# roboterax/humanoid-gym

Hardware: AMD Instinct MI355X
Metric: env-steps/s (XBot-L PPO, whole job) (higher is better)
Workload: dtype bf16

## Files before the change

### humanoid-gym_amd/csrc/hgym_fused.hpp

```cpp
#pragma once
#include "hgym_finalize.hpp"
#pragma clang fp contract(fast)
#include "hgym_gemm.hpp"

namespace hgym {

constexpr int FUSED_CHUNK = 128;

struct __attribute__((packed, aligned(4))) F4 {
    float v[4];
};
typedef __attribute__((ext_vector_type(4))) short s16x4;
typedef __attribute__((ext_vector_type(2))) unsigned int u32x2;

struct FusedLayer {
    const u32x4* Wf;
    const u32x4* WTf;
    const float* bias;
    int K, N;
    int KB;
    int NB;
    int NBB;
};

// ... 607 lines not shown
        stage_load(c0);
        hook_early(extra);
        stage_write(c0, 0);
        bias_to_lds();
        if constexpr (PART) {
#pragma unroll
            for (int i = 0; i < MB; ++i)
#pragma unroll
                for (int g = 0; g < G1; ++g)
#pragma unroll
                    for (int e = 0; e < 4; ++e) acc[i][g][e] = drop[i] ? 0.0f : acc[i][g][e];
        }
        __syncthreads();
        phase_stamp(a.dbg, 1);
        for (int c = c0; c + 1 < NC; ++c) {
            stage_load(c + 1);
            mma_chunk<G1, MB, D, false, XBF>(r0, wl0, L0.KB * 64, (c - c0) * 4, Q + ((c - c0) & 1) * (BM * FUSED_CHUNK * 2), 8, lane, acc);
            stage_write(c + 1, (c + 1 - c0) & 1);
            __syncthreads();
        }
        mma_chunk<G1, MB, D, true, XBF>(r0, wl0, L0.KB * 64, (NC - 1 - c0) * 4, Q + ((NC - 1 - c0) & 1) * (BM * FUSED_CHUNK * 2), 8, lane, acc);
        phase_stamp(a.dbg, 2);
        if (AHEAD) prime1();
        epilogue_elu<G1, MB, GA>(acc, bl, nb0, P, L0.NB, train_h ? n.H[0] : nullptr, mbg0, lane, a.act);
    }
    __syncthreads();
    phase_stamp(a.dbg, 3);
    hook_mid(extra);
    if (!AHEAD) prime1();
    auto prime2 = [&]() { hidden_prime<GH, D>(r2, L2, wave, lane); };
    hidden_layer<GH, MB, NW, D, AHEAD, GA>(r1, L1, bl + L0.N, P, L0.NB, Q, train_h ? n.H[1] : nullptr, mbg0, wave, lane, prime2, a.act);
    __syncthreads();
    phase_stamp(a.dbg, 4);
    if (!AHEAD) prime2();
    WRing<1, 4> r3;
    auto prime3 = [&]() {
        if (wave < MB) wring_prime<1, 4>(r3, L3.Wf + lane, 0, L3.KB);
    };
    hidden_layer<GH, MB, NW, D, AHEAD, GA>(r2, L2, bl + L0.N + L1.N, Q, L1.NB, PH2, train_h ? n.H[2] : nullptr, mbg0, wave, lane, prime3, a.act);
    if (wave * GH >= L2.NB) hook_l2idle(extra);
    __syncthreads();
    phase_stamp(a.dbg, 5);
    if (!AHEAD) prime3();
    if (wave < MB) {
        f32x4 hacc[1][1];
        hacc[0][0] = (f32x4){0.f, 0.f, 0.f, 0.f};
        const int CB3 = L2.NB;
        if (L3.KB % 4 == 0) mma_stream<1, 1, 4>(r3, L3.Wf + lane, 0, L3.KB, PH2 + wave * CB3 * 512, CB3, lane, hacc);
        else mma_ring<1, 1, 4>(r3, L3.Wf + lane, 0, 0, L3.KB, L3.KB, PH2 + wave * CB3 * 512, CB3, lane, hacc);
        const f32x4 acc = hacc[0][0];
        const int m = m0 + wave * 16 + r;
        const int No = L3.N;
        float mu[4];
#pragma unroll
        for (int e = 0; e < 4; ++e) mu[e] = acc[e] + ((4 * q + e < No) ? bl[L0.N + L1.N + L2.N + 4 * q + e] : 0.0f);
        if (m < a.M && n.out) {
#pragma unroll
            for (int e = 0; e < 4; ++e)
                if (4 * q + e < No) n.out[(int64_t)m * n.ldo + 4 * q + e] = mu[e];
        }
        hook_head(wave, m, 0, mu);
        if (is_actor && a.sample) {
#pragma clang fp contract(off)
            const int A = a.A;
            float zz[4];
            if (a.z) {
#pragma unroll
                for (int e = 0; e < 4; ++e) zz[e] = (m < a.M && 4 * q + e < A) ? a.z[(int64_t)m * A + 4 * q + e] : 0.0f;
            } else {
                const int64_t s = HOIST ? step_pre : (a.step ? a.step[0] : 0);
                const RngKey rk = {a.k0, a.k1, (uint32_t)s, (uint32_t)(s >> 32)};
                const U4 u = rng4(rk, (uint32_t)m, SLOT_POLICY + (uint32_t)q);
                box_muller(u.x, u.y, zz[0], zz[1]);
                box_muller(u.z, u.w, zz[2], zz[3]);
            }
            float lp = 0.0f;
#pragma unroll
            for (int e = 0; e < 4; ++e) {
                const int j = 4 * q + e;
                if (j < A) {
                    const float sg = mu[e] * 0.0f + (HOIST ? std_pre[e] : a.std_[j]);
                    const float act = mu[e] + sg * zz[e];
                    const float d = act - mu[e];
                    lp += -(d * d) / (2.0f * sg * sg) - (HOIST ? lsg_pre[e] : log_sigma(sg)) - 0.9189385332046727f;
                    if (m < a.M) {
                        a.actions[(int64_t)m * A + j] = act;
                        a.sigma[(int64_t)m * A + j] = sg;
                    }
                    hook_put(wave * 16 + r, j, act);
                }
            }
            lp += __shfl_xor(lp, 16, 64);
            lp += __shfl_xor(lp, 32, 64);
            if (q == 0 && m < a.M) a.logp[m] = lp;
        }
        for (int nb = 1; WIDE && nb < L3.NB; ++nb) {
            const u32x4* wl = L3.Wf + (int64_t)nb * L3.KB * 64 + lane;
            wring_prime<1, 4>(r3, wl, 0, L3.KB);
            hacc[0][0] = (f32x4){0.f, 0.f, 0.f, 0.f};
            if (L3.KB % 4 == 0) mma_stream<1, 1, 4>(r3, wl, 0, L3.KB, PH2 + wave * CB3 * 512, CB3, lane, hacc);
            else mma_ring<1, 1, 4>(r3, wl, 0, 0, L3.KB, L3.KB, PH2 + wave * CB3 * 512, CB3, lane, hacc);
            float y[4];
#pragma unroll
            for (int e = 0; e < 4; ++e) {
                const int col = nb * 16 + 4 * q + e;
                y[e] = hacc[0][0][e] + (col < No ? bl[L0.N + L1.N + L2.N + col] : 0.0f);
            }
            if (m < a.M && n.out) {
#pragma unroll
                for (int e = 0; e < 4; ++e)
                    if (nb * 16 + 4 * q + e < No) n.out[(int64_t)m * n.ldo + nb * 16 + 4 * q + e] = y[e];
            }
            hook_head(wave, m, nb, y);
        }
    } else {
        hook_idle(extra);
    }
    phase_stamp(a.dbg, 6);
}

template <int BM, int NW, int D, bool FIN = false>
__global__ __launch_bounds__(NW * 64) void mlp_fwd_kernel(const FwdArgs a) {
    extern __shared__ __attribute__((aligned(16))) char smem[];
    if (FIN && (int)blockIdx.y >= a.nets) {
        if (blockIdx.x == 0) fin_block(a.fin, threadIdx.x, NW * 64);
        return;
    }
    const int which = a.net0 + blockIdx.y;
    const FusedNet& n = a.net[which];
    const int g1 = n.layer[0].NB / NW;
    constexpr int U = 16 / NW;
    if (n.layer[3].NB > 1) {
        if (g1 == 2 * U) fwd_body<BM, NW, D, 2 * U, true>(a, n, false, smem);
        return;
    }
    if (g1 == 2 * U) fwd_body<BM, NW, D, 2 * U>(a, n, which == 0, smem);
    else if (g1 == 3 * U) fwd_body<BM, NW, D, 3 * U>(a, n, which == 0, smem);
    else if (g1 == U) fwd_body<BM, NW, D, U>(a, n, which == 0, smem);
}

template <int BM, int NW, int D, int G1U, bool WIDE>
__global__ __launch_bounds__(NW * 64) void mlp_fwd_act_kernel(const FwdArgs a) {
    extern __shared__ __attribute__((aligned(16))) char smem[];
    constexpr int U = 16 / NW;
    fwd_body<BM, NW, D, G1U * U, WIDE, false, false, true>(a, a.net[a.net0], !WIDE && a.net0 == 0, smem);
}

template <int G, int D, int GR>
__device__ __forceinline__ void bwd_prime(WRing<GR, D>& R, const u32x4* __restrict__ WTf, int NBo, int NBBc, int wave, int lane) {
    const int nb0 = wave * G;
    if (nb0 < NBo) wring_prime<G, D>(R, WTf + (int64_t)nb0 * NBBc * 64 + lane, NBBc * 64, NBBc);
}

template <int G, int MB, int NW, int D, bool AHEAD, bool HLDS = false, bool GA = false, int GR, class Next>
__device__ __forceinline__ void bwd_step(WRing<GR, D>& R, const u32x4* __restrict__ WTf, int NBo, int NBBc, const char* in_lds, int CBin,
                                         char* out_lds, __bf16* __restrict__ dZg, const __bf16* __restrict__ Hg, int64_t mbg0, int wave,
                                         int lane, Next prime_next, const char* H_lds = nullptr, const Act* fn = nullptr) {
    const int r = lane & 15, q = lane >> 4;
    float d0p = 0.f, d1p = 0.f, d0n = 0.f, d1n = 0.f, ndq = 0.f;
    if constexpr (GA) { d0p = fn->d0p; d1p = fn->d1p; d0n = fn->d0n; d1n = fn->d1n; ndq = -fn->dq; }
    const int loff = r * 32 + q * 8;
    bool primed = false;
    for (int nb0 = wave * G; nb0 < NBo; nb0 += NW * G) {
        f32x4 acc[MB][G];
        zero_acc<G, MB>(acc);
        if (NBBc % D == 0) mma_stream<G, MB, D>(R, WTf + (int64_t)nb0 * NBBc * 64 + lane, NBBc * 64, NBBc, in_lds, CBin, lane, acc);
        else mma_ring<G, MB, D>(R, WTf + (int64_t)nb0 * NBBc * 64 + lane, NBBc * 64, 0, NBBc, NBBc, in_lds, CBin, lane, acc);
        const int nxt = nb0 + NW * G;
        if (nxt < NBo) wring_prime<G, D>(R, WTf + (int64_t)nxt * NBBc * 64 + lane, NBBc * 64, NBBc);
        else if (AHEAD) { prime_next(); primed = true; }
        u32x2 aux[MB][G];
#pragma unroll
        for (int i = 0; i < MB; ++i)
#pragma unroll
            for (int g = 0; g < G; ++g) {
                if (HLDS) aux[i][g] = *reinterpret_cast<const u32x2*>(H_lds + (i * NBo + nb0 + g) * 512 + loff);
                else aux[i][g] = ld_stream_u2<(kFusedNT & 4) != 0>(reinterpret_cast<const char*>(Hg) + ((mbg0 + i) * NBo + nb0 + g) * 512 + loff);
            }
        static_assert(MB % 2 == 0, "row blocks are stored in pairs");
#pragma unroll
        for (int i = 0; i < MB; i += 2)
#pragma unroll
            for (int g = 0; g < G; ++g) {
                u32x2 pk[2];
#pragma unroll
                for (int h = 0; h < 2; ++h) {
                    const unsigned int w0 = aux[i + h][g][0], w1 = aux[i + h][g][1];
                    const float y[4] = {bf16_bits_to_f32(w0 & 0xffffu), bf16_bits_to_f32(w0 >> 16), bf16_bits_to_f32(w1 & 0xffffu),
                                        bf16_bits_to_f32(w1 >> 16)};
                    float d[4];
                    if constexpr (GA) {
#pragma unroll
                        for (int e = 0; e < 4; ++e) {
                            const bool p = y[e] > 0.0f;
                            d[e] = acc[i + h][g][e] * fmaf(y[e], fmaf(ndq, y[e], p ? d1p : d1n), p ? d0p : d0n);
                        }
                    } else {
#pragma unroll
                        for (int e = 0; e < 4; ++e) d[e] = acc[i + h][g][e] * ((y[e] > 0.0f) ? 1.0f : (y[e] + 1.0f));
                    }
                    pk[h] = pack_bf16x4(d[0], d[1], d[2], d[3]);
                    if (out_lds) *reinterpret_cast<u32x2*>(out_lds + ((i + h) * NBo + nb0 + g) * 512 + loff) = pk[h];
                }
                char* pa = reinterpret_cast<char*>(dZg) + ((mbg0 + i) * NBo + nb0 + g) * 512 + loff;
                st_pair<(kFusedNT & 4) != 0, false>(pa, pa + (int64_t)NBo * 512, pk[0], pk[1], true, true, q);
            }
    }
    if (AHEAD && !primed) prime_next();
}

struct FbLoss {
    const float* actions;
    const float* old_mu;
    const float* old_sigma;
    const float* values;
    const float* advantages;
    const float* returns;
    const float* logp;
    float clip, value_coef, entropy_coef;
    float* partials;
    const float* aux_target;
    int64_t aux_ldt;
    int aux_off;
    float aux_coef;
};

constexpr int FB_LIN_ACTOR = 40;
HG_HD int fb_lds_lin(const FusedNet& n) { return n.layer[3].N == 1 ? 64 * 2 * 4 : (n.layer[3].N <= 12 ? 64 * FB_LIN_ACTOR * 4 : 0); }
HG_HD int fb_lds_extra(const FusedNet& n) { return 64 * 64 * n.layer[3].NBB + 4 * 32 * 4 + 64 * n.layer[2].N * 2 + 256 + fb_lds_lin(n); }

constexpr size_t FB_LDS_LIMIT = 160 * 1024;
HG_HD int fwd_lds_bytes(const FusedNet& n, int BM) { return fused_lds_p(n, BM) + fused_lds_q(n, BM) + fused_lds_bias(n); }
HG_HD int fb_lds_bytes(const FusedNet& n) { return fwd_lds_bytes(n, 64) + fb_lds_extra(n); }
inline int fb_lds_bytes(const int32_t* dims) {
    FusedNet n{};
    for (int l = 0; l < 4; ++l) {
        n.layer[l].K = dims[l];
        n.layer[l].N = dims[l + 1];
        n.layer[l].NB = (dims[l + 1] + 15) / 16;
        n.layer[l].NBB = (dims[l + 1] + 31) / 32;
    }
    return fb_lds_bytes(n);
}

template <int G1, bool AUX = false, bool XB16 = false, bool VU = false, bool GA = false>
__device__ __forceinline__ void fb_body(const FwdArgs& a, const FbLoss& L, const FusedNet& n, bool is_actor, char* smem) {
    constexpr int BM = 64, NW = 16, D = 2, MB = BM / 16;
    const int tid = threadIdx.x, lane = tid & 63, wave = tid >> 6;
    const int r = lane & 15, q = lane >> 4;
    const int m0 = blockIdx.x * BM;
    const int64_t mbg0 = m0 >> 4;
    char* P = smem;
    char* Q = smem + fused_lds_p(n, BM);
    char* R0 = smem + fused_lds_p(n, BM) + fused_lds_q(n, BM) + fused_lds_bias(n);
    const int NBB3 = n.layer[3].NBB, CB3 = 2 * NBB3;
    float* red = reinterpret_cast<float*>(R0 + BM * 64 * NBB3);
    char* H2 = R0 + BM * 64 * NBB3 + 4 * 32 * 4;
    int* rowidx = reinterpret_cast<int*>(H2 + BM * n.layer[2].N * 2);
    float* lin = reinterpret_cast<float*>(rowidx + BM);
    const int A = a.A;
    const bool pre = !AUX && n.layer[2].NB <= 8 && (is_actor ? A == 12 : true);
    const float invB = 1.0f / (float)a.M;
    float aux_se = 0.0f;
    auto head_aux = [&](int hw, int m, int nb, const float (&out)[4]) {
        const int No = n.layer[3].N;
        const bool valid = m < a.M;
        const int64_t row = rowidx[hw * 16 + r];
        const float* t = L.aux_target + row * L.aux_ldt + L.aux_off;
        const float gs = 2.0f * L.aux_coef / ((float)a.M * (float)No);
        float g[4];
#pragma unroll
        for (int e = 0; e < 4; ++e) {
            const int j = nb * 16 + 4 * q + e;
            float d = 0.0f;
            if (valid && j < No) {
                d = out[e] - t[j];
                aux_se += d * d;
            }
            g[e] = gs * d;
        }
        const u32x2 pk = pack_bf16x4(g[0], g[1], g[2], g[3]);
        const int off = (hw * CB3 + nb) * 512 + r * 32 + q * 8;
        char* gz = reinterpret_cast<char*>(n.dZ[3]) + mbg0 * CB3 * 512;
        *reinterpret_cast<u32x2*>(R0 + off) = pk;
        *reinterpret_cast<u32x2*>(gz + off) = pk;
        if (nb == 0) {
            const u32x2 zero = {0u, 0u};
            for (int cb = n.layer[3].NB; cb < CB3; ++cb) {
                const int offz = (hw * CB3 + cb) * 512 + r * 32 + q * 8;
                *reinterpret_cast<u32x2*>(R0 + offz) = zero;
                *reinterpret_cast<u32x2*>(gz + offz) = zero;
            }
        }
    };
    auto l2idle = [&](int) {
        if (!pre) return;
        const int j = tid - 8 * 64;
        if (j < 0) return;
        if (is_actor) {
            const int rw = j >> 3, k = j & 7;
            const int64_t ri = rowidx[rw];
            const float* base = k < 3 ? L.actions : (k < 6 ? L.old_mu : L.old_sigma);
            const F4 v1 = *reinterpret_cast<const F4*>(base + ri * 12 + 4 * (k < 3 ? k : (k < 6 ? k - 3 : k - 6)));
            const int rw2 = j & 63;
            const int64_t ri2 = rowidx[rw2];
            const F4 v2 = *reinterpret_cast<const F4*>(L.old_sigma + ri2 * 12 + 8);
            const float s2 = (j < 128 ? L.advantages : L.logp)[ri2];
            *reinterpret_cast<F4*>(lin + rw * FB_LIN_ACTOR + 4 * k) = v1;
            if (j < 64) *reinterpret_cast<F4*>(lin + rw2 * FB_LIN_ACTOR + 32) = v2;
            else if (j < 192) lin[rw2 * FB_LIN_ACTOR + (j < 128 ? 36 : 37)] = s2;
        } else if (j < 128) {
            const int rw = j & 63;
            const int64_t ri = rowidx[rw];
            lin[rw * 2 + (j >> 6)] = j < 64 ? L.returns[ri] : L.values[ri];
        }
    };
    auto head = [&](int hw, int m, int, const float (&out)[4]) {
        const bool valid = m < a.M;
        const int rl = hw * 16 + r;
        const int64_t row = rowidx[rl];
        float g[4] = {0.f, 0.f, 0.f, 0.f};
        float part[11];
#pragma unroll
        for (int k = 0; k < 11; ++k) part[k] = 0.0f;
        if (is_actor) {
            float act[4] = {0.f, 0.f, 0.f, 0.f}, mo[4] = {0.f, 0.f, 0.f, 0.f}, so[4] = {1.f, 1.f, 1.f, 1.f}, sg[4] = {1.f, 1.f, 1.f, 1.f};
            if (pre) {
                if (q < 3) {
                    const F4 qa = *reinterpret_cast<const F4*>(lin + rl * FB_LIN_ACTOR + 4 * q);
                    const F4 qo = *reinterpret_cast<const F4*>(lin + rl * FB_LIN_ACTOR + 12 + 4 * q);
                    const F4 qs = *reinterpret_cast<const F4*>(lin + rl * FB_LIN_ACTOR + 24 + 4 * q);
#pragma unroll
                    for (int e = 0; e < 4; ++e) { act[e] = qa.v[e]; mo[e] = qo.v[e]; so[e] = qs.v[e]; }
                }
            } else if (4 * q + 3 < A) {
                const F4 qa = *reinterpret_cast<const F4*>(L.actions + row * A + 4 * q);
                const F4 qo = *reinterpret_cast<const F4*>(L.old_mu + row * A + 4 * q);
                const F4 qs = *reinterpret_cast<const F4*>(L.old_sigma + row * A + 4 * q);
#pragma unroll
                for (int e = 0; e < 4; ++e) { act[e] = qa.v[e]; mo[e] = qo.v[e]; so[e] = qs.v[e]; }
            } else {
#pragma unroll
                for (int e = 0; e < 4; ++e)
                    if (4 * q + e < A) { act[e] = L.actions[row * A + 4 * q + e]; mo[e] = L.old_mu[row * A + 4 * q + e]; so[e] = L.old_sigma[row * A + 4 * q + e]; }
            }
            const float adv = pre ? lin[rl * FB_LIN_ACTOR + 36] : L.advantages[row], lpold = pre ? lin[rl * FB_LIN_ACTOR + 37] : L.logp[row];
            float lp = 0.0f, ent = 0.0f, kl = 0.0f, diff[4];
#pragma unroll
            for (int e = 0; e < 4; ++e) {
                diff[e] = 0.0f;
                if (4 * q + e < A) {
                    const float mm = out[e];
                    const float s = mm * 0.0f + a.std_[4 * q + e];
                    const float d = act[e] - mm;
                    diff[e] = d;
                    sg[e] = s;
                    lp += -(d * d) / (2.0f * s * s) - logf(s) - 0.9189385332046727f;
                    ent += 0.5f + 0.9189385332046727f + logf(s);
                    kl += logf(s / so[e] + 1.e-5f) + (so[e] * so[e] + (mo[e] - mm) * (mo[e] - mm)) / (2.0f * (s * s)) - 0.5f;
                }
            }
            lp += __shfl_xor(lp, 16, 64);  lp += __shfl_xor(lp, 32, 64);
            ent += __shfl_xor(ent, 16, 64); ent += __shfl_xor(ent, 32, 64);
            kl += __shfl_xor(kl, 16, 64);  kl += __shfl_xor(kl, 32, 64);
            const float ratio = expf(lp - lpold);
            const float s1 = -adv * ratio;
            const float s2 = -adv * clampf(ratio, 1.0f - L.clip, 1.0f + L.clip);
            const float in_range = (ratio >= 1.0f - L.clip && ratio <= 1.0f + L.clip) ? 1.0f : 0.0f;
            const float w1 = s1 > s2 ? 1.0f : (s1 == s2 ? 0.5f : 0.0f);
            const float d_lp = (-adv) * (w1 + (1.0f - w1) * in_range) * invB * ratio;
            if (valid) {
                if (q == 0) { part[0] = fmaxf(s1, s2); part[1] = ent; part[2] = kl; }
#pragma unroll
                for (int e = 0; e < 4; ++e)
                    if (4 * q + e < A) {
                        const float s = sg[e], d = diff[e];
                        g[e] = d_lp * d / (s * s);
                        part[3 + e] = d_lp * (d * d / (s * s * s) - 1.0f / s) - (L.entropy_coef * invB) / s;
                        part[7 + e] = g[e];
                    }
            }
        } else {
            const float ret = pre ? lin[rl * 2] : L.returns[row], vold = pre ? lin[rl * 2 + 1] : L.values[row];
            const float v = out[0];
            if constexpr (VU) {
                (void)vold;
                if (valid && q == 0) {
                    g[0] = L.value_coef * invB * (2.0f * (v - ret));
                    part[0] = (v - ret) * (v - ret);
                    part[1] = g[0];
                }
            } else {
                const float vc = vold + clampf(v - vold, -L.clip, L.clip);
                const float l1 = (v - ret) * (v - ret), l2 = (vc - ret) * (vc - ret);
                const float v_in = ((v - vold) >= -L.clip && (v - vold) <= L.clip) ? 1.0f : 0.0f;
                const float u1 = l1 > l2 ? 1.0f : (l1 == l2 ? 0.5f : 0.0f);
                if (valid && q == 0) {
                    g[0] = L.value_coef * invB * (u1 * 2.0f * (v - ret) + (1.0f - u1) * 2.0f * (vc - ret) * v_in);
                    part[0] = fmaxf(l1, l2);
                    part[1] = g[0];
                }
            }
        }
        const u32x2 pk = pack_bf16x4(g[0], g[1], g[2], g[3]);
        const u32x2 zero = {0u, 0u};
        const int off0 = (hw * 2 + 0) * 512 + r * 32 + q * 8, off1 = (hw * 2 + 1) * 512 + r * 32 + q * 8;
        *reinterpret_cast<u32x2*>(R0 + off0) = pk;
        *reinterpret_cast<u32x2*>(R0 + off1) = zero;
        char* gz = reinterpret_cast<char*>(n.dZ[3]) + mbg0 * 2 * 512;
        *reinterpret_cast<u32x2*>(gz + off0) = pk;
        *reinterpret_cast<u32x2*>(gz + off1) = zero;
#pragma unroll
        for (int k = 0; k < 11; ++k) {
            float v = part[k];
            v += __shfl_xor(v, 1, 64); v += __shfl_xor(v, 2, 64); v += __shfl_xor(v, 4, 64); v += __shfl_xor(v, 8, 64);
            part[k] = v;
        }
        if (r == 0) {
            float* w = red + hw * 32;
            if (is_actor) {
                if (q == 0) { w[0] = part[0]; w[2] = part[1]; w[3] = part[2]; }
#pragma unroll
                for (int e = 0; e < 4; ++e)
                    if (4 * q + e < 12) { w[4 + 4 * q + e] = part[3 + e]; w[16 + 4 * q + e] = part[7 + e]; }
            } else if (q == 0) {
                w[1] = part[0];
                w[28] = part[1];
            }
        }
    };
    if constexpr (AUX) {
        fwd_body<BM, NW, D, G1, true, XB16, false, GA>(a, n, false, smem, FwdNoop(), FwdNoop(), FwdNoop(), 0, FwdNoop(), head_aux, H2, rowidx);
        if (wave < MB) {
#pragma unroll
            for (int o = 32; o > 0; o >>= 1) aux_se += __shfl_xor(aux_se, o, 64);
            if (lane == 0) red[wave * 32 + 29] = aux_se;
        }
    } else {
        fwd_body<BM, NW, D, G1, false, XB16, false, GA>(a, n, is_actor, smem, FwdNoop(), FwdNoop(), FwdNoop(), 0, FwdNoop(), head, H2, rowidx, l2idle);
    }
    __syncthreads();
    if (tid < 32) {
        const bool mine = AUX ? tid == 29 : (is_actor ? (tid != 1 && tid < 28) : (tid == 1 || tid == 28));
        if (mine) L.partials[(int64_t)blockIdx.x * 32 + tid] = red[tid] + red[32 + tid] + red[64 + tid] + red[96 + tid];
    }
    const int N0 = n.layer[0].N, N1 = n.layer[1].N, N2 = n.layer[2].N;
    WRing<1, D> ra;
    WRing<1, D> rb;
    WRing<G1, D> rc;
    auto none = [&]() {};
    bwd_prime<1, D>(ra, n.layer[3].WTf, N2 / 16, NBB3, wave, lane);
    bwd_step<1, MB, NW, D, false, true, GA>(ra, n.layer[3].WTf, N2 / 16, NBB3, R0, 2 * NBB3, H2, n.dZ[2], nullptr, mbg0, wave, lane, none, H2, &a.act);
    __syncthreads();
    bwd_prime<1, D>(rb, n.layer[2].WTf, N1 / 16, n.layer[2].NBB, wave, lane);
    bwd_step<1, MB, NW, D, false, true, GA>(rb, n.layer[2].WTf, N1 / 16, n.layer[2].NBB, H2, N2 / 16, Q, n.dZ[1], nullptr, mbg0, wave, lane, none, Q, &a.act);
    __syncthreads();
    bwd_prime<G1, D>(rc, n.layer[1].WTf, N0 / 16, n.layer[1].NBB, wave, lane);
    bwd_step<G1, MB, NW, D, false, true, GA>(rc, n.layer[1].WTf, N0 / 16, n.layer[1].NBB, Q, N1 / 16, nullptr, n.dZ[0], nullptr, mbg0, wave, lane, none, P, &a.act);
    phase_stamp(a.dbg, 7);
}

template <bool XB16 = false, bool VU = false>
__global__ __launch_bounds__(1024) void mlp_fb_kernel(const FwdArgs a, const FbLoss L) {
    extern __shared__ __attribute__((aligned(16))) char smem[];
    const int which = a.net0 + blockIdx.y;
    const FusedNet& n = a.net[which];
    const int g1 = n.layer[0].NB / 16;
    if (which == 2) {
        if (g1 == 2) fb_body<2, true, XB16, VU>(a, L, n, false, smem);
        return;
    }
    if (g1 == 2) fb_body<2, false, XB16, VU>(a, L, n, which == 0, smem);
    else if (g1 == 3) fb_body<3, false, XB16, VU>(a, L, n, which == 0, smem);
    else if (g1 == 1) fb_body<1, false, XB16, VU>(a, L, n, which == 0, smem);
}

template <bool VU>
int32_t launch_mlp_fb_form(const FwdArgs& fb, const FbLoss& fl, bool shadow, int tiles, int nets, size_t lds, hipStream_t s) {
    const int32_t rc = shadow ? ensure_dynamic_lds(reinterpret_cast<const void*>(&mlp_fb_kernel<true, VU>), lds, "mlp_fb_kernel<shadow>")
                              : ensure_dynamic_lds(reinterpret_cast<const void*>(&mlp_fb_kernel<false, VU>), lds, "mlp_fb_kernel");
    if (rc) return rc;
    if (shadow) hipLaunchKernelGGL((mlp_fb_kernel<true, VU>), dim3(tiles, nets), dim3(1024), lds, s, fb, fl);
    else hipLaunchKernelGGL((mlp_fb_kernel<false, VU>), dim3(tiles, nets), dim3(1024), lds, s, fb, fl);
    return HGYM_OK;
}

template <int G1, bool AUX, bool XB16, bool VU>
__global__ __launch_bounds__(1024) void mlp_fb_act_kernel(const FwdArgs a, const FbLoss L) {
    extern __shared__ __attribute__((aligned(16))) char smem[];
    fb_body<G1, AUX, XB16, VU, true>(a, L, a.net[a.net0], !AUX && a.net0 == 0, smem);
}

template <int G1, bool AUX, bool VU>
int32_t launch_mlp_fb_act_one(const FwdArgs& fb, const FbLoss& fl, bool shadow, int tiles, size_t lds, hipStream_t s) {
    const int32_t rc = shadow ? ensure_dynamic_lds(reinterpret_cast<const void*>(&mlp_fb_act_kernel<G1, AUX, true, VU>), lds, "mlp_fb_act_kernel<shadow>")
                              : ensure_dynamic_lds(reinterpret_cast<const void*>(&mlp_fb_act_kernel<G1, AUX, false, VU>), lds, "mlp_fb_act_kernel");
    if (rc) return rc;
    if (shadow) hipLaunchKernelGGL((mlp_fb_act_kernel<G1, AUX, true, VU>), dim3(tiles), dim3(1024), lds, s, fb, fl);
    else hipLaunchKernelGGL((mlp_fb_act_kernel<G1, AUX, false, VU>), dim3(tiles), dim3(1024), lds, s, fb, fl);
    return HGYM_OK;
}
template <bool VU>
int32_t launch_mlp_fb_act_form(const FwdArgs& fb0, const FbLoss& fl, bool shadow, int tiles, int nets, hipStream_t s) {
    for (int i = 0; i < nets; ++i) {
        FwdArgs fb = fb0;
        fb.net0 = i;
        fb.nets = 1;
        if (fb.dbg) fb.dbg += (int64_t)i * tiles * 8;
        const size_t lds = (size_t)fb_lds_bytes(fb.net[i]);
        const int g1 = fb.net[i].layer[0].NB / 16;
        int32_t rc = HGYM_E_UNSUPPORTED;
        if (i == 2) rc = launch_mlp_fb_act_one<2, true, VU>(fb, fl, shadow, tiles, lds, s);
        else if (g1 == 1) rc = launch_mlp_fb_act_one<1, false, VU>(fb, fl, shadow, tiles, lds, s);
        else if (g1 == 2) rc = launch_mlp_fb_act_one<2, false, VU>(fb, fl, shadow, tiles, lds, s);
        else if (g1 == 3) rc = launch_mlp_fb_act_one<3, false, VU>(fb, fl, shadow, tiles, lds, s);
        if (rc) return rc;
    }
    return HGYM_OK;
}

constexpr int LOSS_PARTIALS = 32;
struct ScalArgs {
    int nblocks, B, A, aux_No;
    const float* partials;
    float* grads_std;
    float* grads_bmu;
    float* grads_bv;
    float* kl_slot;
    double* opt;
    double beta1, beta2;
    int do_prologue, adaptive_lr;
    float desired_kl;
    double lr_min, lr_max;
    int group;
};
__device__ __forceinline__ double adapt_lr(double lr, float kl, float desired_kl, double lr_min, double lr_max) {
    if (kl > desired_kl * 2.0f) return fmax(lr_min, lr / 1.5);
    if (kl < desired_kl * 0.5f && kl > 0.0f) return fmin(lr_max, lr * 1.5);
    return lr;
}
__device__ __forceinline__ void ppo_scalars_block(const ScalArgs& a, int tid, int nthreads) {
    __shared__ double red[16][LOSS_PARTIALS + 1];
    if (tid >= nthreads - 2 && !(a.opt[13] == a.opt[1] && a.opt[1] > 0.0)) {
        const double t = a.opt[1] + 1.0;
        const double pw = pow(tid == nthreads - 2 ? a.beta1 : a.beta2, t);
        a.opt[tid == nthreads - 2 ? 14 : 15] = pw;
        if (tid == nthreads - 2) a.opt[13] = t;
    }
    const float* __restrict__ partials = a.partials;
    const int nblocks = a.nblocks, B = a.B, A = a.A;
    const int k = tid & (LOSS_PARTIALS - 1);
    for (int part = tid / LOSS_PARTIALS; part < 16; part += nthreads / LOSS_PARTIALS) {
        double s0 = 0.0, s1 = 0.0, s2 = 0.0, s3 = 0.0;
        int b = part;
        if (a.group == 4) {
            auto ld = [&](int g) -> float {
                const float* p = partials + (int64_t)g * 4 * LOSS_PARTIALS + k;
                const float p0 = p[0], p1 = p[LOSS_PARTIALS], p2 = p[2 * LOSS_PARTIALS], p3 = p[3 * LOSS_PARTIALS];
                return ((p0 + p1) + p2) + p3;
            };
            for (; b + 48 < nblocks; b += 64) {
                const float v0 = ld(b), v1 = ld(b + 16), v2 = ld(b + 32), v3 = ld(b + 48);
                s0 += (double)v0; s1 += (double)v1; s2 += (double)v2; s3 += (double)v3;
            }
            for (; b < nblocks; b += 16) s0 += (double)ld(b);
        } else {
            for (; b + 48 < nblocks; b += 64) {
                const float v0 = partials[(int64_t)b * LOSS_PARTIALS + k], v1 = partials[(int64_t)(b + 16) * LOSS_PARTIALS + k];
                const float v2 = partials[(int64_t)(b + 32) * LOSS_PARTIALS + k], v3 = partials[(int64_t)(b + 48) * LOSS_PARTIALS + k];
                s0 += (double)v0; s1 += (double)v1; s2 += (double)v2; s3 += (double)v3;
            }
            for (; b < nblocks; b += 16) s0 += (double)partials[(int64_t)b * LOSS_PARTIALS + k];
        }
        red[part][k] = (s0 + s1) + (s2 + s3);
    }
    __syncthreads();
    if (tid < LOSS_PARTIALS) {
        double t = 0.0;
        for (int p = 0; p < 16; ++p) t += red[p][tid];
        const int q = tid;
        double* __restrict__ opt = a.opt;
        if (q == 0) opt[3] += t / B;
        if (q == 1) opt[4] += t / B;
        if (q == 2) opt[5] += t / B;
        if (q == 3) {
            const float kl = (float)(t / B);
            opt[2] += t / B;
            opt[8] = (double)kl;
            opt[7] += 1.0;
            opt[9] = 0.0;
            a.kl_slot[0] = kl;
            if (a.do_prologue && !(opt[13] == opt[1] && opt[1] > 0.0)) {
                double lr = opt[0];
                if (a.adaptive_lr) {
                    lr = adapt_lr(lr, kl, a.desired_kl, a.lr_min, a.lr_max);
                    opt[0] = lr;
                }
                const double ts = opt[1] + 1.0;
                opt[1] = ts;
                const double bc1 = 1.0 - opt[14], bc2 = 1.0 - opt[15];
                opt[11] = (double)(float)(lr / bc1);
                opt[12] = (double)(float)sqrt(bc2);
            }
        }
        if (q >= 4 && q < 16 && q - 4 < A) a.grads_std[q - 4] = (float)t;
        if (q >= 16 && q < 28 && q - 16 < A && a.grads_bmu) a.grads_bmu[q - 16] = (float)t;
        if (q == 28 && a.grads_bv) a.grads_bv[0] = (float)t;
        if (q == 29 && a.aux_No > 0) opt[10] += t / ((double)B * (double)a.aux_No);
    }
}

constexpr int DW_THREADS = 512;
constexpr int DW_Z_BYTES = 8192;
constexpr int DW_STAGE_BYTES = 24576;
constexpr int DW_LDS_STAGES = 3;
constexpr int DW_TILE_N = 128, DW_TILE_K = 256;
constexpr int DW_MAX_PRODUCTS = 12;

struct DwProduct {
    const __bf16* Z;
    const __bf16* X;
    const int64_t* gidx;
    int64_t ldg;
    int CBz, CBx;
    int N, K;
    int64_t w_off;
    int64_t b_off;
    int tiles_n, tiles_k, tile0;
};

struct DwArgs {
    DwProduct p[DW_MAX_PRODUCTS];
    int np;
    int total_tiles;
    int splits;
    int steps_total;
    int steps_per_split;
    float* slabs;
    int64_t slab_stride;
    const char* zeros;
    int B;
    int scal_bid;
    ScalArgs sc;
};

__device__ __forceinline__ u32x4 tr_frag(const char* p0, const char* p1) {
    typedef s16x4 __attribute__((address_space(3)))* lds_p;
    const s16x4 a = __builtin_amdgcn_ds_read_tr16_b64_v4i16((lds_p)(const_cast<char*>(p0)));
    const s16x4 b = __builtin_amdgcn_ds_read_tr16_b64_v4i16((lds_p)(const_cast<char*>(p1)));
    struct { s16x4 a, b; } pr = {a, b};
    return __builtin_bit_cast(u32x4, pr);
}

template <int DW_RS>
__global__ __launch_bounds__(DW_THREADS, 1) void dw_kernel_rs(const DwArgs a) {
    static_assert(DW_RS == 3, "ring indices below: three register stages over three LDS stages, unrolled by six");
    extern __shared__ __attribute__((aligned(16))) char smem[];
    const int tid = threadIdx.x, lane = tid & 63, wave = tid >> 6;
    const int wi = wave >> 1, wj = wave & 1;
    const int r = lane & 15, q = lane >> 4;
    const int bid = blockIdx.x;
    if (bid == a.scal_bid) {
        ppo_scalars_block(a.sc, tid, DW_THREADS);
        return;
    }
    const int xcd = bid & 7, slot = bid >> 3;
    const int split = xcd + 8 * (slot / a.total_tiles);
    const int tile = slot % a.total_tiles;
// ... 157 lines not shown
```

### humanoid-gym_amd/csrc/hgym_update.hip

```cpp
#include "hgym_fused.hpp"

namespace hgym {

int32_t launch_mlp_fb_unclipped(const FwdArgs& fb, const FbLoss& fl, bool shadow, int tiles, int nets, size_t lds, hipStream_t s);

int32_t launch_mlp_fb(const FwdArgs& fb, const FbLoss& fl, bool shadow, bool unclipped, int tiles, int nets, size_t lds, hipStream_t s) {
    if (unclipped) return launch_mlp_fb_unclipped(fb, fl, shadow, tiles, nets, lds, s);
    return launch_mlp_fb_form<false>(fb, fl, shadow, tiles, nets, lds, s);
}

}
```

### humanoid-gym_amd/csrc/hgym_update_act.hip

```cpp
#include "hgym_fused.hpp"

namespace hgym {

int32_t launch_mlp_fb_act_unclipped(const FwdArgs& fb, const FbLoss& fl, bool shadow, int tiles, int nets, hipStream_t s);

int32_t launch_mlp_fb_act(const FwdArgs& fb, const FbLoss& fl, bool shadow, bool unclipped, int tiles, int nets, hipStream_t s) {
    if (unclipped) return launch_mlp_fb_act_unclipped(fb, fl, shadow, tiles, nets, s);
    return launch_mlp_fb_act_form<false>(fb, fl, shadow, tiles, nets, s);
}

}
```

Measured before the change: 42.14 million.

## Fuse last-layer backward into loss head and prefetch next backward weights

For the PPO fused forward/backward kernel, the output layer's dZ computation (a single-block MMA against preloaded transposed head weights) is moved into the per-wave loss head, so it is no longer a separate backward step behind a block barrier. While the forward pass is idle, the weight ring for the next backward layer is primed, and the first-layer ring priming is chained into the second step for small G1. This is meant to shorten the serialized backward tail and remove one __syncthreads. It adds register pressure (eight held weight fragments) and an env-gated fallback path built in separate translation units for shapes that do not match.

```diff
diff --git a/humanoid-gym_amd/csrc/hgym_fused.hpp b/humanoid-gym_amd/csrc/hgym_fused.hpp
--- a/humanoid-gym_amd/csrc/hgym_fused.hpp
+++ b/humanoid-gym_amd/csrc/hgym_fused.hpp
@@ -783,13 +783,39 @@
     if (nb0 < NBo) wring_prime<G, D>(R, WTf + (int64_t)nb0 * NBBc * 64 + lane, NBBc * 64, NBBc);
 }
 
+struct ActD {
+    float d0p, d1p, d0n, d1n, ndq;
+};
+template <bool GA>
+__device__ __forceinline__ ActD act_d(const Act* fn) {
+    ActD k = {0.f, 0.f, 0.f, 0.f, 0.f};
+    if constexpr (GA) { k.d0p = fn->d0p; k.d1p = fn->d1p; k.d0n = fn->d0n; k.d1n = fn->d1n; k.ndq = -fn->dq; }
+    return k;
+}
+template <bool GA>
+__device__ __forceinline__ u32x2 dz_block(const f32x4& acc, u32x2 y2, const ActD& k) {
+    const unsigned int w0 = y2[0], w1 = y2[1];
+    const float y[4] = {bf16_bits_to_f32(w0 & 0xffffu), bf16_bits_to_f32(w0 >> 16), bf16_bits_to_f32(w1 & 0xffffu), bf16_bits_to_f32(w1 >> 16)};
+    float d[4];
+    if constexpr (GA) {
+#pragma unroll
+        for (int e = 0; e < 4; ++e) {
+            const bool p = y[e] > 0.0f;
+            d[e] = acc[e] * fmaf(y[e], fmaf(k.ndq, y[e], p ? k.d1p : k.d1n), p ? k.d0p : k.d0n);
+        }
+    } else {
+#pragma unroll
+        for (int e = 0; e < 4; ++e) d[e] = acc[e] * ((y[e] > 0.0f) ? 1.0f : (y[e] + 1.0f));
+    }
+    return pack_bf16x4(d[0], d[1], d[2], d[3]);
+}
+
 template <int G, int MB, int NW, int D, bool AHEAD, bool HLDS = false, bool GA = false, int GR, class Next>
 __device__ __forceinline__ void bwd_step(WRing<GR, D>& R, const u32x4* __restrict__ WTf, int NBo, int NBBc, const char* in_lds, int CBin,
                                          char* out_lds, __bf16* __restrict__ dZg, const __bf16* __restrict__ Hg, int64_t mbg0, int wave,
                                          int lane, Next prime_next, const char* H_lds = nullptr, const Act* fn = nullptr) {
     const int r = lane & 15, q = lane >> 4;
-    float d0p = 0.f, d1p = 0.f, d0n = 0.f, d1n = 0.f, ndq = 0.f;
-    if constexpr (GA) { d0p = fn->d0p; d1p = fn->d1p; d0n = fn->d0n; d1n = fn->d1n; ndq = -fn->dq; }
+    const ActD dk = act_d<GA>(fn);
     const int loff = r * 32 + q * 8;
     bool primed = false;
     for (int nb0 = wave * G; nb0 < NBo; nb0 += NW * G) {
@@ -816,21 +842,7 @@
                 u32x2 pk[2];
 #pragma unroll
                 for (int h = 0; h < 2; ++h) {
-                    const unsigned int w0 = aux[i + h][g][0], w1 = aux[i + h][g][1];
-                    const float y[4] = {bf16_bits_to_f32(w0 & 0xffffu), bf16_bits_to_f32(w0 >> 16), bf16_bits_to_f32(w1 & 0xffffu),
-                                        bf16_bits_to_f32(w1 >> 16)};
-                    float d[4];
-                    if constexpr (GA) {
-#pragma unroll
-                        for (int e = 0; e < 4; ++e) {
-                            const bool p = y[e] > 0.0f;
-                            d[e] = acc[i + h][g][e] * fmaf(y[e], fmaf(ndq, y[e], p ? d1p : d1n), p ? d0p : d0n);
-                        }
-                    } else {
-#pragma unroll
-                        for (int e = 0; e < 4; ++e) d[e] = acc[i + h][g][e] * ((y[e] > 0.0f) ? 1.0f : (y[e] + 1.0f));
-                    }
-                    pk[h] = pack_bf16x4(d[0], d[1], d[2], d[3]);
+                    pk[h] = dz_block<GA>(acc[i + h][g], aux[i + h][g], dk);
                     if (out_lds) *reinterpret_cast<u32x2*>(out_lds + ((i + h) * NBo + nb0 + g) * 512 + loff) = pk[h];
                 }
                 char* pa = reinterpret_cast<char*>(dZg) + ((mbg0 + i) * NBo + nb0 + g) * 512 + loff;
@@ -874,8 +886,24 @@
     return fb_lds_bytes(n);
 }
 
-template <int G1, bool AUX = false, bool XB16 = false, bool VU = false, bool GA = false>
+HG_HD bool fb_tail_ok(const FusedNet& n, bool is_actor, int A) { return n.layer[3].NBB == 1 && n.layer[2].NB == 8 && (is_actor ? A == 12 : true); }
+inline bool fb_tail_launch_ok(const FwdArgs& fb, int nets) {
+    const char* v = getenv("HGYM_FB_TAIL");
+    if (v && v[0] == '0') return false;
+    for (int i = 0; i < nets && i < 2; ++i)
+        if (!fb_tail_ok(fb.net[fb.net0 + i], fb.net0 + i == 0, fb.A)) return false;
+    return true;
+}
+
+#ifdef HGYM_FB_TAIL_CLOCK
+#define HG_TAIL_STAMP(slot) phase_stamp(a.dbg, slot)
+#else
+#define HG_TAIL_STAMP(slot)
+#endif
+
+template <int G1, bool AUX = false, bool XB16 = false, bool VU = false, bool GA = false, bool TAIL = true>
 __device__ __forceinline__ void fb_body(const FwdArgs& a, const FbLoss& L, const FusedNet& n, bool is_actor, char* smem) {
+    constexpr bool TA = TAIL && !AUX;
     constexpr int BM = 64, NW = 16, D = 2, MB = BM / 16;
     const int tid = threadIdx.x, lane = tid & 63, wave = tid >> 6;
     const int r = lane & 15, q = lane >> 4;
@@ -890,7 +918,16 @@
     int* rowidx = reinterpret_cast<int*>(H2 + BM * n.layer[2].N * 2);
     float* lin = reinterpret_cast<float*>(rowidx + BM);
     const int A = a.A;
-    const bool pre = !AUX && n.layer[2].NB <= 8 && (is_actor ? A == 12 : true);
+    const bool pre = !AUX && (TA || (n.layer[2].NB <= 8 && (is_actor ? A == 12 : true)));
+    const int N0 = n.layer[0].N, N1 = n.layer[1].N, N2 = n.layer[2].N;
+    WRing<1, D> rb;
+    WRing<G1, D> rc;
+    constexpr int NB2 = 8;
+    u32x4 w3t[TA ? NB2 : 1];
+    auto prime_b = [&]() { bwd_prime<1, D>(rb, n.layer[2].WTf, N1 / 16, n.layer[2].NBB, wave, lane); };
+    auto idle_ta = [&](int) { prime_b(); };
+    const ActD dk = act_d<GA>(&a.act);
+    (void)w3t; (void)idle_ta; (void)dk;
     const float invB = 1.0f / (float)a.M;
     float aux_se = 0.0f;
     auto head_aux = [&](int hw, int m, int nb, const float (&out)[4]) {
@@ -954,6 +991,18 @@
         float part[11];
 #pragma unroll
         for (int k = 0; k < 11; ++k) part[k] = 0.0f;
+        float sd[4] = {1.f, 1.f, 1.f, 1.f};
+        if constexpr (TA) {
+            if (is_actor) {
+#pragma unroll
+                for (int e = 0; e < 4; ++e) sd[e] = a.std_[4 * q + e < A ? 4 * q + e : 0];
+            }
+            __builtin_amdgcn_sched_barrier(0);
+#pragma unroll
+            for (int gb = 0; gb < NB2; ++gb) w3t[gb] = n.layer[3].WTf[gb * 64 + lane];
+            prime_b();
+            __builtin_amdgcn_sched_barrier(0);
+        }
         if (is_actor) {
             float act[4] = {0.f, 0.f, 0.f, 0.f}, mo[4] = {0.f, 0.f, 0.f, 0.f}, so[4] = {1.f, 1.f, 1.f, 1.f}, sg[4] = {1.f, 1.f, 1.f, 1.f};
             if (pre) {
@@ -982,7 +1031,7 @@
                 diff[e] = 0.0f;
                 if (4 * q + e < A) {
                     const float mm = out[e];
-                    const float s = mm * 0.0f + a.std_[4 * q + e];
+                    const float s = mm * 0.0f + (TA ? sd[e] : a.std_[4 * q + e]);
                     const float d = act[e] - mm;
                     diff[e] = d;
                     sg[e] = s;
@@ -1059,6 +1108,23 @@
                 w[28] = part[1];
             }
         }
+        if constexpr (TA) {
+            const int loff = r * 32 + q * 8;
+            asm volatile("" ::: "memory");
+            const u32x4 x = *reinterpret_cast<const u32x4*>(R0 + (q >> 1) * 512 + r * 32 + (q & 1) * 16 + (hw * 2) * 512);
+            u32x2 y2[NB2];
+#pragma unroll
+            for (int gb = 0; gb < NB2; ++gb) y2[gb] = *reinterpret_cast<const u32x2*>(H2 + (hw * NB2 + gb) * 512 + loff);
+            char* gd = reinterpret_cast<char*>(n.dZ[2]) + (mbg0 + hw) * NB2 * 512 + loff;
+#pragma unroll
+            for (int gb = 0; gb < NB2; ++gb) {
+                f32x4 acc = (f32x4){0.f, 0.f, 0.f, 0.f};
+                mma_frag<__bf16>(w3t[gb], x, acc);
+                const u32x2 pk2 = dz_block<GA>(acc, y2[gb], dk);
+                *reinterpret_cast<u32x2*>(H2 + (hw * NB2 + gb) * 512 + loff) = pk2;
+                st_stream_u2<(kFusedNT & 4) != 0>(gd + gb * 512, pk2);
+            }
+        }
     };
     if constexpr (AUX) {
         fwd_body<BM, NW, D, G1, true, XB16, false, GA>(a, n, false, smem, FwdNoop(), FwdNoop(), FwdNoop(), 0, FwdNoop(), head_aux, H2, rowidx);
@@ -1067,71 +1133,84 @@
             for (int o = 32; o > 0; o >>= 1) aux_se += __shfl_xor(aux_se, o, 64);
             if (lane == 0) red[wave * 32 + 29] = aux_se;
         }
+    } else if constexpr (TA) {
+        fwd_body<BM, NW, D, G1, false, XB16, false, GA>(a, n, is_actor, smem, FwdNoop(), FwdNoop(), FwdNoop(), 0, idle_ta, head, H2, rowidx, l2idle);
     } else {
         fwd_body<BM, NW, D, G1, false, XB16, false, GA>(a, n, is_actor, smem, FwdNoop(), FwdNoop(), FwdNoop(), 0, FwdNoop(), head, H2, rowidx, l2idle);
     }
     __syncthreads();
+    HG_TAIL_STAMP(1);
     if (tid < 32) {
         const bool mine = AUX ? tid == 29 : (is_actor ? (tid != 1 && tid < 28) : (tid == 1 || tid == 28));
         if (mine) L.partials[(int64_t)blockIdx.x * 32 + tid] = red[tid] + red[32 + tid] + red[64 + tid] + red[96 + tid];
     }
-    const int N0 = n.layer[0].N, N1 = n.layer[1].N, N2 = n.layer[2].N;
-    WRing<1, D> ra;
-    WRing<1, D> rb;
-    WRing<G1, D> rc;
     auto none = [&]() {};
-    bwd_prime<1, D>(ra, n.layer[3].WTf, N2 / 16, NBB3, wave, lane);
-    bwd_step<1, MB, NW, D, false, true, GA>(ra, n.layer[3].WTf, N2 / 16, NBB3, R0, 2 * NBB3, H2, n.dZ[2], nullptr, mbg0, wave, lane, none, H2, &a.act);
-    __syncthreads();
-    bwd_prime<1, D>(rb, n.layer[2].WTf, N1 / 16, n.layer[2].NBB, wave, lane);
-    bwd_step<1, MB, NW, D, false, true, GA>(rb, n.layer[2].WTf, N1 / 16, n.layer[2].NBB, H2, N2 / 16, Q, n.dZ[1], nullptr, mbg0, wave, lane, none, Q, &a.act);
-    __syncthreads();
-    bwd_prime<G1, D>(rc, n.layer[1].WTf, N0 / 16, n.layer[1].NBB, wave, lane);
+    auto prime_c = [&]() { bwd_prime<G1, D>(rc, n.layer[1].WTf, N0 / 16, n.layer[1].NBB, wave, lane); };
+    if constexpr (TA) {
+        HG_TAIL_STAMP(2);
+        constexpr bool CA = G1 <= 2;
+        bwd_step<1, MB, NW, D, CA, true, GA>(rb, n.layer[2].WTf, N1 / 16, n.layer[2].NBB, H2, N2 / 16, Q, n.dZ[1], nullptr, mbg0, wave, lane, prime_c, Q, &a.act);
+        HG_TAIL_STAMP(3);
+        __syncthreads();
+        if (!CA) prime_c();
+    } else {
+        WRing<1, D> ra;
+        bwd_prime<1, D>(ra, n.layer[3].WTf, N2 / 16, NBB3, wave, lane);
+        bwd_step<1, MB, NW, D, false, true, GA>(ra, n.layer[3].WTf, N2 / 16, NBB3, R0, 2 * NBB3, H2, n.dZ[2], nullptr, mbg0, wave, lane, none, H2, &a.act);
+        __syncthreads();
+        HG_TAIL_STAMP(2);
+        prime_b();
+        bwd_step<1, MB, NW, D, false, true, GA>(rb, n.layer[2].WTf, N1 / 16, n.layer[2].NBB, H2, N2 / 16, Q, n.dZ[1], nullptr, mbg0, wave, lane, none, Q, &a.act);
+        HG_TAIL_STAMP(3);
+        __syncthreads();
+        prime_c();
+    }
+    HG_TAIL_STAMP(4);
     bwd_step<G1, MB, NW, D, false, true, GA>(rc, n.layer[1].WTf, N0 / 16, n.layer[1].NBB, Q, N1 / 16, nullptr, n.dZ[0], nullptr, mbg0, wave, lane, none, P, &a.act);
     phase_stamp(a.dbg, 7);
 }
 
-template <bool XB16 = false, bool VU = false>
+template <bool XB16 = false, bool VU = false, bool TAIL = true>
 __global__ __launch_bounds__(1024) void mlp_fb_kernel(const FwdArgs a, const FbLoss L) {
     extern __shared__ __attribute__((aligned(16))) char smem[];
     const int which = a.net0 + blockIdx.y;
     const FusedNet& n = a.net[which];
     const int g1 = n.layer[0].NB / 16;
     if (which == 2) {
-        if (g1 == 2) fb_body<2, true, XB16, VU>(a, L, n, false, smem);
+        if (g1 == 2) fb_body<2, true, XB16, VU, false, TAIL>(a, L, n, false, smem);
         return;
     }
-    if (g1 == 2) fb_body<2, false, XB16, VU>(a, L, n, which == 0, smem);
-    else if (g1 == 3) fb_body<3, false, XB16, VU>(a, L, n, which == 0, smem);
-    else if (g1 == 1) fb_body<1, false, XB16, VU>(a, L, n, which == 0, smem);
-}
-
-template <bool VU>
+    if (g1 == 2) fb_body<2, false, XB16, VU, false, TAIL>(a, L, n, which == 0, smem);
+    else if (g1 == 3) fb_body<3, false, XB16, VU, false, TAIL>(a, L, n, which == 0, smem);
+    else if (g1 == 1) fb_body<1, false, XB16, VU, false, TAIL>(a, L, n, which == 0, smem);
+}
+
+template <bool VU, bool TAIL = true>
 int32_t launch_mlp_fb_form(const FwdArgs& fb, const FbLoss& fl, bool shadow, int tiles, int nets, size_t lds, hipStream_t s) {
-    const int32_t rc = shadow ? ensure_dynamic_lds(reinterpret_cast<const void*>(&mlp_fb_kernel<true, VU>), lds, "mlp_fb_kernel<shadow>")
-                              : ensure_dynamic_lds(reinterpret_cast<const void*>(&mlp_fb_kernel<false, VU>), lds, "mlp_fb_kernel");
+    const int32_t rc = shadow ? ensure_dynamic_lds(reinterpret_cast<const void*>(&mlp_fb_kernel<true, VU, TAIL>), lds, "mlp_fb_kernel<shadow>")
+                              : ensure_dynamic_lds(reinterpret_cast<const void*>(&mlp_fb_kernel<false, VU, TAIL>), lds, "mlp_fb_kernel");
     if (rc) return rc;
-    if (shadow) hipLaunchKernelGGL((mlp_fb_kernel<true, VU>), dim3(tiles, nets), dim3(1024), lds, s, fb, fl);
-    else hipLaunchKernelGGL((mlp_fb_kernel<false, VU>), dim3(tiles, nets), dim3(1024), lds, s, fb, fl);
+    if (shadow) hipLaunchKernelGGL((mlp_fb_kernel<true, VU, TAIL>), dim3(tiles, nets), dim3(1024), lds, s, fb, fl);
+    else hipLaunchKernelGGL((mlp_fb_kernel<false, VU, TAIL>), dim3(tiles, nets), dim3(1024), lds, s, fb, fl);
     return HGYM_OK;
 }
 
-template <int G1, bool AUX, bool XB16, bool VU>
+template <int G1, bool AUX, bool XB16, bool VU, bool TAIL = true>
 __global__ __launch_bounds__(1024) void mlp_fb_act_kernel(const FwdArgs a, const FbLoss L) {
     extern __shared__ __attribute__((aligned(16))) char smem[];
-    fb_body<G1, AUX, XB16, VU, true>(a, L, a.net[a.net0], !AUX && a.net0 == 0, smem);
-}
-
-template <int G1, bool AUX, bool VU>
+    fb_body<G1, AUX, XB16, VU, true, TAIL>(a, L, a.net[a.net0], !AUX && a.net0 == 0, smem);
+}
+
+template <int G1, bool AUX, bool VU, bool TAIL>
 int32_t launch_mlp_fb_act_one(const FwdArgs& fb, const FbLoss& fl, bool shadow, int tiles, size_t lds, hipStream_t s) {
-    const int32_t rc = shadow ? ensure_dynamic_lds(reinterpret_cast<const void*>(&mlp_fb_act_kernel<G1, AUX, true, VU>), lds, "mlp_fb_act_kernel<shadow>")
-                              : ensure_dynamic_lds(reinterpret_cast<const void*>(&mlp_fb_act_kernel<G1, AUX, false, VU>), lds, "mlp_fb_act_kernel");
+    const int32_t rc = shadow ? ensure_dynamic_lds(reinterpret_cast<const void*>(&mlp_fb_act_kernel<G1, AUX, true, VU, TAIL>), lds, "mlp_fb_act_kernel<shadow>")
+                              : ensure_dynamic_lds(reinterpret_cast<const void*>(&mlp_fb_act_kernel<G1, AUX, false, VU, TAIL>), lds, "mlp_fb_act_kernel");
     if (rc) return rc;
-    if (shadow) hipLaunchKernelGGL((mlp_fb_act_kernel<G1, AUX, true, VU>), dim3(tiles), dim3(1024), lds, s, fb, fl);
-    else hipLaunchKernelGGL((mlp_fb_act_kernel<G1, AUX, false, VU>), dim3(tiles), dim3(1024), lds, s, fb, fl);
+    if (shadow) hipLaunchKernelGGL((mlp_fb_act_kernel<G1, AUX, true, VU, TAIL>), dim3(tiles), dim3(1024), lds, s, fb, fl);
+    else hipLaunchKernelGGL((mlp_fb_act_kernel<G1, AUX, false, VU, TAIL>), dim3(tiles), dim3(1024), lds, s, fb, fl);
     return HGYM_OK;
 }
-template <bool VU>
+template <bool VU, bool TAIL = true>
 int32_t launch_mlp_fb_act_form(const FwdArgs& fb0, const FbLoss& fl, bool shadow, int tiles, int nets, hipStream_t s) {
     for (int i = 0; i < nets; ++i) {
         FwdArgs fb = fb0;
@@ -1141,10 +1220,10 @@
         const size_t lds = (size_t)fb_lds_bytes(fb.net[i]);
         const int g1 = fb.net[i].layer[0].NB / 16;
         int32_t rc = HGYM_E_UNSUPPORTED;
-        if (i == 2) rc = launch_mlp_fb_act_one<2, true, VU>(fb, fl, shadow, tiles, lds, s);
-        else if (g1 == 1) rc = launch_mlp_fb_act_one<1, false, VU>(fb, fl, shadow, tiles, lds, s);
-        else if (g1 == 2) rc = launch_mlp_fb_act_one<2, false, VU>(fb, fl, shadow, tiles, lds, s);
-        else if (g1 == 3) rc = launch_mlp_fb_act_one<3, false, VU>(fb, fl, shadow, tiles, lds, s);
+        if (i == 2) rc = launch_mlp_fb_act_one<2, true, VU, TAIL>(fb, fl, shadow, tiles, lds, s);
+        else if (g1 == 1) rc = launch_mlp_fb_act_one<1, false, VU, TAIL>(fb, fl, shadow, tiles, lds, s);
+        else if (g1 == 2) rc = launch_mlp_fb_act_one<2, false, VU, TAIL>(fb, fl, shadow, tiles, lds, s);
+        else if (g1 == 3) rc = launch_mlp_fb_act_one<3, false, VU, false>(fb, fl, shadow, tiles, lds, s);
         if (rc) return rc;
     }
     return HGYM_OK;
diff --git a/humanoid-gym_amd/csrc/hgym_update.hip b/humanoid-gym_amd/csrc/hgym_update.hip
--- a/humanoid-gym_amd/csrc/hgym_update.hip
+++ b/humanoid-gym_amd/csrc/hgym_update.hip
@@ -3,8 +3,10 @@
 namespace hgym {
 
 int32_t launch_mlp_fb_unclipped(const FwdArgs& fb, const FbLoss& fl, bool shadow, int tiles, int nets, size_t lds, hipStream_t s);
+int32_t launch_mlp_fb_tail0(const FwdArgs& fb, const FbLoss& fl, bool shadow, bool unclipped, int tiles, int nets, size_t lds, hipStream_t s);
 
 int32_t launch_mlp_fb(const FwdArgs& fb, const FbLoss& fl, bool shadow, bool unclipped, int tiles, int nets, size_t lds, hipStream_t s) {
+    if (!fb_tail_launch_ok(fb, nets)) return launch_mlp_fb_tail0(fb, fl, shadow, unclipped, tiles, nets, lds, s);
     if (unclipped) return launch_mlp_fb_unclipped(fb, fl, shadow, tiles, nets, lds, s);
     return launch_mlp_fb_form<false>(fb, fl, shadow, tiles, nets, lds, s);
 }
diff --git a/humanoid-gym_amd/csrc/hgym_update_act.hip b/humanoid-gym_amd/csrc/hgym_update_act.hip
--- a/humanoid-gym_amd/csrc/hgym_update_act.hip
+++ b/humanoid-gym_amd/csrc/hgym_update_act.hip
@@ -3,8 +3,10 @@
 namespace hgym {
 
 int32_t launch_mlp_fb_act_unclipped(const FwdArgs& fb, const FbLoss& fl, bool shadow, int tiles, int nets, hipStream_t s);
+int32_t launch_mlp_fb_act_tail0(const FwdArgs& fb, const FbLoss& fl, bool shadow, bool unclipped, int tiles, int nets, hipStream_t s);
 
 int32_t launch_mlp_fb_act(const FwdArgs& fb, const FbLoss& fl, bool shadow, bool unclipped, int tiles, int nets, hipStream_t s) {
+    if (!fb_tail_launch_ok(fb, nets)) return launch_mlp_fb_act_tail0(fb, fl, shadow, unclipped, tiles, nets, s);
     if (unclipped) return launch_mlp_fb_act_unclipped(fb, fl, shadow, tiles, nets, s);
     return launch_mlp_fb_act_form<false>(fb, fl, shadow, tiles, nets, s);
 }
diff --git a/humanoid-gym_amd/csrc/hgym_update_act_tail0.hip b/humanoid-gym_amd/csrc/hgym_update_act_tail0.hip
--- /dev/null
+++ b/humanoid-gym_amd/csrc/hgym_update_act_tail0.hip
@@ -0,0 +1,10 @@
+#include "hgym_fused.hpp"
+
+namespace hgym {
+
+int32_t launch_mlp_fb_act_tail0(const FwdArgs& fb, const FbLoss& fl, bool shadow, bool unclipped, int tiles, int nets, hipStream_t s) {
+    if (unclipped) return launch_mlp_fb_act_form<true, false>(fb, fl, shadow, tiles, nets, s);
+    return launch_mlp_fb_act_form<false, false>(fb, fl, shadow, tiles, nets, s);
+}
+
+}
diff --git a/humanoid-gym_amd/csrc/hgym_update_tail0.hip b/humanoid-gym_amd/csrc/hgym_update_tail0.hip
--- /dev/null
+++ b/humanoid-gym_amd/csrc/hgym_update_tail0.hip
@@ -0,0 +1,10 @@
+#include "hgym_fused.hpp"
+
+namespace hgym {
+
+int32_t launch_mlp_fb_tail0(const FwdArgs& fb, const FbLoss& fl, bool shadow, bool unclipped, int tiles, int nets, size_t lds, hipStream_t s) {
+    if (unclipped) return launch_mlp_fb_form<true, false>(fb, fl, shadow, tiles, nets, lds, s);
+    return launch_mlp_fb_form<false, false>(fb, fl, shadow, tiles, nets, lds, s);
+}
+
+}
```

New measurement: 42.43 million, median of 6. Within noise of the previous version (+0.7%).
